# zxhuang1698/ShapeClipper

Hardware: AMD Instinct MI355X
Metric: train-step images/sec (Pix3D cfg, bs32/GPU) (higher is better)
Workload: dtype f32 (bf16x3-split MFMA, fp32 accumulate)

## Files before the change

shapeclipper_amd/csrc/conv3x3.hip:

```cpp
#include <hip/hip_runtime.h>

#include <map>
#include <mutex>
#include <tuple>
#include <vector>

#include "grid_cus.hpp"
#include "shapeclipper_hip.h"

#ifndef SC_CONV_SPANS
#define SC_CONV_SPANS 1
#endif
#ifndef SC_CONV_ABLATE
#define SC_CONV_ABLATE 0
#endif

namespace sc {

#ifdef SC_CONV_PROFILE
__device__ unsigned long long* conv_prof_buf = nullptr;
#define CV_STAMP(ID) { const unsigned long long t_ = __builtin_amdgcn_s_memrealtime(); if (conv_prof_buf && tid == 0) conv_prof_buf[(size_t)g * 32 + (ID)] = t_; }
#else
#define CV_STAMP(ID)
#endif

typedef float f32x16 __attribute__((ext_vector_type(16)));
typedef __bf16 cv_bf16x8 __attribute__((ext_vector_type(8)));
typedef __bf16 cv_bf16x2 __attribute__((ext_vector_type(2)));
typedef __attribute__((address_space(3))) void* lptr_cv_t;

__device__ __forceinline__ void conv_glds16(const void* gsrc, unsigned lds_dst) {
    unsigned keep;
    asm volatile("s_mov_b32 %0, m0\n\ts_mov_b32 m0, %2\n\ts_nop 0\n\tglobal_load_lds_dwordx4 %1, off\n\ts_mov_b32 m0, %0"
                 : "=&s"(keep) : "v"(gsrc), "s"(lds_dst) : "memory");
}

template <int W_, int CT_, int PT_, int WGM_, int WGN_, bool SPLIT_ = false, int S_ = 1, bool BD2_ = false>
struct ConvCfg {
    static constexpr int W = W_, CT = CT_, PT = PT_, WGM = WGM_, WGN = WGN_, CB = 8;
    static constexpr bool SPLIT = SPLIT_;
    static constexpr bool BD2 = BD2_;
    static constexpr int PSZ = 3 * 2 * CT * 4;
    static constexpr bool PAIRED = SPLIT && !BD2_;
    static_assert(!BD2 || (SPLIT && S_ == 1), "the stride-2 backward-data instance exists in the split arithmetic only");
    static constexpr int Wp = W + 2, HW = W * W, Sp = Wp * Wp;
    static constexpr int S = S_, WO = W / S, HWO = WO * WO;
    static constexpr int NT = 64 * WGM * WGN;
    static constexpr int WM = CT / (32 * WGM), WN = PT / (32 * WGN);
    static constexpr int WIMG = BD2 ? 2 * PSZ : (SPLIT ? 5 * PSZ : 9 * CB * CT);
    static constexpr int LMAX = S == 1 ? PT + 2 * (PT / W + 2) + 2 * Wp * (PT / HW + 1) + 2 * (Wp + 1)
                                       : S * PT + (PT / WO + 2) * S * (Wp - WO) + (PT / HWO + 1) * (Sp - S * (WO - 1) * (Wp + 1)) + 2 * (Wp + 1);
    static constexpr int LX = LMAX;
    static constexpr int NXE = (LMAX + NT - 1) / NT;
    static constexpr int STAGE = WIMG + (SPLIT ? 3 : 2) * LX * 4;
    static constexpr int LDS_BYTES = 2 * STAGE * 4;
    static constexpr int TILE = CT * PT;
    static constexpr int WGS_PER_CU = NT == 512 ? 1 : 2;
    static_assert(WM >= 1 && WN >= 1 && (NT == 512 || NT == 256) && LDS_BYTES * WGS_PER_CU <= 160 * 1024, "tile shape");
};

template <class C>
__device__ __forceinline__ int padded_q(int p) {
    const int b = p / C::HWO, r = p - b * C::HWO, y = r / C::WO, x = r - y * C::WO;
    return b * C::Sp + (C::S * y + 1) * C::Wp + (C::S * x + 1);
}

__host__ __device__ constexpr int bd2_pairs(int phase) { return phase == 3 ? 2 : 1; }
__host__ __device__ constexpr int bd2_pair_base(int phase) { return phase; }
__host__ __device__ constexpr int bd2_filter_tap(int phase, int pair, int h) {
    return phase == 0 ? (h == 0 ? 4 : -1)
         : phase == 1 ? (h == 0 ? 3 : 5)
         : phase == 2 ? (h == 0 ? 1 : 7)
         : pair == 0 ? (h == 0 ? 0 : 2) : (h == 0 ? 6 : 8);
}
__host__ __device__ constexpr int bd2_patch_tap(int phase, int pair, int h) {
    return phase == 0 ? 4
         : phase == 1 ? (h == 0 ? 5 : 4)
         : phase == 2 ? (h == 0 ? 7 : 4)
         : pair == 0 ? (h == 0 ? 8 : 7) : (h == 0 ? 5 : 4);
}

template <class C>
__host__ __device__ constexpr int conv_nk(int cin) { return C::PAIRED ? ((cin / C::CB + 1) & ~1) : cin / C::CB; }

struct ConvSplit {
    int rounds;
    int tail_tiles;
    int per_wg;
};
__host__ __device__ inline ConvSplit conv_split(int tiles, int nk, int G) {
    ConvSplit s;
    s.rounds = tiles / G;
    s.tail_tiles = tiles - s.rounds * G;
    s.per_wg = (int)(((long long)s.tail_tiles * nk + G - 1) / G);
    return s;
}

__device__ __forceinline__ long long conv_span_at(const int* __restrict__ spans, const ConvSplit& sp, int g, int nk) {
    return spans ? (long long)spans[g] : min((long long)g * sp.per_wg, (long long)sp.tail_tiles * nk);
}
__device__ __forceinline__ int conv_span_owner(const int* __restrict__ spans, const ConvSplit& sp, long long u, int G) {
    if (!spans) return (int)(u / sp.per_wg);
    int lo = 0, hi = G - 1;
    while (lo < hi) {
        const int mid = (lo + hi + 1) >> 1;
        if (spans[mid] <= u) lo = mid; else hi = mid - 1;
    }
    return lo;
}

template <class C>
__device__ __forceinline__ void conv_tile_decode(int tile, int nct, int& phase, int& pt, int& ct) {
    phase = C::BD2 ? tile & 3 : 0;
    const int t = C::BD2 ? tile >> 2 : tile;
    pt = t / nct, ct = t - pt * nct;
}
template <class C>
__device__ __forceinline__ float* conv_out_pixel(float* __restrict__ out, int p, int phase, int cout, int& cstride) {
    const int b = p / C::HWO, rem = p - b * C::HWO;
    if constexpr (C::BD2) {
        const int y = rem / C::W, x = rem - y * C::W;
        cstride = 4 * C::HW;
        return out + (size_t)b * cout * cstride + (2 * y + (phase >> 1)) * (2 * C::W) + 2 * x + (phase & 1);
    } else {
        cstride = C::HWO;
        return out + (size_t)b * cout * C::HWO + rem;
    }
}

template <class C>
__device__ __forceinline__ void conv_store_tile(float* __restrict__ out, const f32x16 (&acc)[C::WM][C::WN], int tile, int nct, int npix,
                                                int cout, int wm, int wn, int lane, const float* __restrict__ addend) {
    int phase, pt, ct;
    conv_tile_decode<C>(tile, nct, phase, pt, ct);
#pragma unroll
    for (int j = 0; j < C::WN; ++j) {
        const int p = pt * C::PT + (wn * C::WN + j) * 32 + (lane & 31);
        if (p >= npix) continue;
        int cs;
        float* ob = conv_out_pixel<C>(out, p, phase, cout, cs);
#pragma unroll
        for (int i = 0; i < C::WM; ++i)
#pragma unroll
            for (int r = 0; r < 16; ++r) {
                const int co = ct * C::CT + (wm * C::WM + i) * 32 + (r & 3) + 8 * (r >> 2) + 4 * (lane >> 5);
                if (co < cout) ob[(size_t)co * cs] = addend ? acc[i][j][r] + addend[(ob - out) + (size_t)co * cs] : acc[i][j][r];
            }
    }
}

template <class C>
__device__ __forceinline__ void conv_split_terms(const float4 (&a)[C::WM][3], const float4 (&b)[C::WN][3], f32x16 (&acc)[C::WM][C::WN]) {
#pragma unroll
    for (int term = 0; term < 6; ++term) {
        constexpr int PA[6] = {0, 2, 1, 0, 1, 0}, PB[6] = {2, 0, 1, 1, 0, 0};
#pragma unroll
        for (int i = 0; i < C::WM; ++i)
#pragma unroll
            for (int j = 0; j < C::WN; ++j)
#if SC_CONV_ABLATE & 1
                acc[i][j][term] += a[i][PA[term]].x * b[j][PB[term]].x;
#else
                acc[i][j] = __builtin_amdgcn_mfma_f32_32x32x16_bf16(__builtin_bit_cast(cv_bf16x8, a[i][PA[term]]),
                                                                    __builtin_bit_cast(cv_bf16x8, b[j][PB[term]]), acc[i][j], 0, 0, 0);
#endif
    }
}
template <class C, int PHASE>
__device__ __forceinline__ void conv_bd2_step(const float* Ws, const float* Xs, const int (&aoff)[C::WM], const int (&boff)[C::WN], int half,
                                              f32x16 (&acc)[C::WM][C::WN]) {
    constexpr int Wp = C::Wp, LX = C::LX, CT = C::CT;
#pragma unroll
    for (int tp = 0; tp < bd2_pairs(PHASE); ++tp) {
        constexpr int dummy = 0;
        (void)dummy;
        const int t0 = bd2_patch_tap(PHASE, tp, 0), t1 = bd2_patch_tap(PHASE, tp, 1);
        const int o0 = (t0 / 3) * Wp + t0 % 3, o1 = (t1 / 3) * Wp + t1 % 3;
        float4 a[C::WM][3], b[C::WN][3];
#pragma unroll
        for (int i = 0; i < C::WM; ++i)
#pragma unroll
            for (int pc = 0; pc < 3; ++pc) a[i][pc] = *reinterpret_cast<const float4*>(Ws + aoff[i] + (tp * 3 + pc) * 2 * CT * 4);
#pragma unroll
        for (int j = 0; j < C::WN; ++j)
#pragma unroll
            for (int pc = 0; pc < 3; ++pc)
                b[j][pc] = *reinterpret_cast<const float4*>(Xs + boff[j] + (pc * LX + o0) * 4 + half * (o1 - o0) * 4);
        conv_split_terms<C>(a, b, acc);
    }
}

template <class C>
__global__ __launch_bounds__(C::NT, C::WGS_PER_CU) void conv3x3_kernel(const float* __restrict__ x, const float* __restrict__ wpack,
                                                             float* __restrict__ out, float* __restrict__ partial, int batch, int cin,
                                                             int cout, const int* __restrict__ spans, const float* __restrict__ addend) {
    constexpr int W = C::W, Wp = C::Wp, HW = C::HW, Sp = C::Sp, CT = C::CT, PT = C::PT, CB = C::CB, NT = C::NT;
    constexpr int WM = C::WM, WN = C::WN, LX = C::LX, NXE = C::NXE;
    extern __shared__ float4 conv_smem[];
    float* S = reinterpret_cast<float*>(conv_smem);
    const int tid = threadIdx.x, lane = tid & 63, wave = tid >> 6, half = lane >> 5;
    const int wm = wave / C::WGN, wn = wave % C::WGN;
    const int npix = batch * C::HWO, nct = (cout + CT - 1) / CT, tiles = ((npix + PT - 1) / PT) * nct * (C::BD2 ? 4 : 1);
    const int nk = conv_nk<C>(cin), nk_real = cin / CB, G = gridDim.x, g = blockIdx.x;
    const ConvSplit sp = conv_split(tiles, nk, G);
    const int xq = G >> 3, xr = G & 7, xcd = g & 7;
    const int gperm = (xcd < xr ? xcd * (xq + 1) : xr * (xq + 1) + (xcd - xr) * xq) + (g >> 3);
    const long long unit_lo = conv_span_at(spans, sp, g, nk), unit_hi = conv_span_at(spans, sp, g + 1, nk);
    const unsigned lds0 = (unsigned)__builtin_amdgcn_readfirstlane((int)(unsigned)(size_t)(lptr_cv_t)S);
    const int wave_u = __builtin_amdgcn_readfirstlane(wave);

    CV_STAMP(0)
    for (int it = 0; it < sp.rounds + 2; ++it) {
        const int item = (C::WGS_PER_CU == 2 && g >= (G >> 1)) ? (it + sp.rounds) % (sp.rounds + 2) : it;
        int tile, kb0, kb1;
        if (item < sp.rounds) {
            tile = item * G + gperm, kb0 = 0, kb1 = nk;
        } else if (item == sp.rounds) {
            if (unit_lo >= unit_hi) continue;
            const int t = (int)(unit_lo / nk);
            tile = sp.rounds * G + t, kb0 = (int)(unit_lo - (long long)t * nk), kb1 = (int)min((long long)nk, unit_hi - (long long)t * nk);
        } else {
            const int t = (int)(unit_lo / nk) + 1;
            if (unit_lo >= unit_hi || (long long)t * nk >= unit_hi) continue;
            tile = sp.rounds * G + t, kb0 = 0, kb1 = (int)(unit_hi - (long long)t * nk);
        }
        int phase, pt, ct;
        conv_tile_decode<C>(tile, nct, phase, pt, ct);
        const int p0 = pt * PT;
        const int q0 = padded_q<C>(p0), q_lo = q0 - Wp - 1;

        int xoff[NXE];
#pragma unroll
        for (int i = 0; i < NXE; ++i) {
            const int e = tid + i * NT, q = q_lo + e;
            const int b = q / Sp, r = q - b * Sp, yp = r / Wp, xp = r - yp * Wp;
            const bool valid = e < C::LMAX && b < batch && yp >= 1 && yp <= W && xp >= 1 && xp <= W;
            xoff[i] = valid ? (b * cin * HW + (yp - 1) * W + (xp - 1)) : -1;
        }
        int boff[WN], aoff[WM];
#pragma unroll
        for (int j = 0; j < WN; ++j) {
            const int p = min(p0 + (wn * WN + j) * 32 + (lane & 31), npix - 1);
            boff[j] = (half * LX + padded_q<C>(p) - q0) * 4;
        }
#pragma unroll
        for (int i = 0; i < WM; ++i) aoff[i] = (half * CT + (wm * WM + i) * 32 + (lane & 31)) * 4;
        if constexpr (C::SPLIT) {
#pragma unroll
            for (int j = 0; j < WN; ++j) boff[j] -= half * LX * 4;
        }

        const int wimg = C::BD2 ? bd2_pairs(phase) * C::PSZ : C::WIMG;
        const float* wsrc = wpack + (C::BD2 ? (size_t)bd2_pair_base(phase) * nct * nk * C::PSZ : 0) +
                            (C::PAIRED ? (size_t)ct * (nk >> 1) * 9 * C::PSZ : (size_t)ct * nk * wimg);
        auto issue_w = [&](int kb, int stage) {
            const int CHUNKS = C::PAIRED ? ((kb & 1) ? 5 : 4) * C::PSZ / 4 : wimg / 4;
            const char* src = reinterpret_cast<const char*>(wsrc + (C::PAIRED ? ((size_t)(kb >> 1) * 9 + (kb & 1) * 4) * C::PSZ : (size_t)kb * wimg));
            const unsigned dst = lds0 + (unsigned)stage * (C::STAGE * 4);
#pragma unroll
            for (int c = 0; c < (C::WIMG / 4 + NT - 1) / NT; ++c) {
                const int chunk0 = c * NT + wave_u * 64;
                if (chunk0 + lane < CHUNKS) conv_glds16(src + (size_t)(chunk0 + lane) * 16, (unsigned)__builtin_amdgcn_readfirstlane((int)(dst + chunk0 * 16)));
            }
        };
        float xv[NXE][CB];
        unsigned xkeep = 0xffffffffu;
        const __amdgpu_buffer_rsrc_t xrs = __builtin_amdgcn_make_buffer_rsrc(
            const_cast<float*>(x), 0, (int)min((long long)batch * cin * HW * 4, 0x7fffffffLL), 0x00020000);
        int xoffb[NXE];
#pragma unroll
        for (int i = 0; i < NXE; ++i) xoffb[i] = xoff[i] >= 0 ? xoff[i] * 4 : (int)0x80000000;
        auto load_x = [&](int kb) {
            if constexpr (C::SPLIT) {
                xkeep = kb < nk_real ? 0xffffffffu : 0u;
#pragma unroll
                for (int i = 0; i < NXE; ++i)
#pragma unroll
                    for (int c = 0; c < CB; ++c)
                        xv[i][c] = __builtin_bit_cast(float, __builtin_amdgcn_raw_buffer_load_b32(xrs, xoffb[i], (kb * CB + c) * HW * 4, 0));
            } else {
                const float* xb = x + (size_t)kb * CB * HW;
#pragma unroll
                for (int i = 0; i < NXE; ++i)
#pragma unroll
                    for (int c = 0; c < CB; ++c) xv[i][c] = xoff[i] >= 0 ? xb[xoff[i] + c * HW] : 0.f;
            }
        };
        auto store_x = [&](int stage) {
            float4* Xs = reinterpret_cast<float4*>(S + stage * C::STAGE + C::WIMG);
#pragma unroll
            for (int i = 0; i < NXE; ++i) {
                const int e = tid + i * NT;
                if (e < C::LMAX) {
                    if constexpr (C::SPLIT) {
                        cv_bf16x8 p0, p1, p2;
#pragma unroll
                        for (int c = 0; c < CB; ++c) {
                            const float v = C::PAIRED ? __uint_as_float(__float_as_uint(xv[i][c]) & xkeep) : xv[i][c];
                            const __bf16 h0 = (__bf16)v;
                            const float r1 = v - (float)h0;
                            const __bf16 h1 = (__bf16)r1;
                            const float r2 = r1 - (float)h1;
                            p0[c] = h0, p1[c] = h1, p2[c] = (__bf16)r2;
                        }
                        Xs[e] = __builtin_bit_cast(float4, p0);
                        Xs[LX + e] = __builtin_bit_cast(float4, p1);
                        Xs[2 * LX + e] = __builtin_bit_cast(float4, p2);
                    } else {
                        Xs[e] = make_float4(xv[i][0], xv[i][1], xv[i][2], xv[i][3]);
                        Xs[LX + e] = make_float4(xv[i][4], xv[i][5], xv[i][6], xv[i][7]);
                    }
                }
            }
        };

        f32x16 acc[WM][WN];
#pragma unroll
        for (int i = 0; i < WM; ++i)
#pragma unroll
            for (int j = 0; j < WN; ++j)
#pragma unroll
                for (int r = 0; r < 16; ++r) acc[i][j][r] = 0.f;

        [[maybe_unused]] const int sid = 1 + 8 * (item < sp.rounds ? 0 : item - sp.rounds + 1);
        CV_STAMP(sid)
        asm volatile("s_waitcnt lgkmcnt(0)\n\ts_barrier" ::: "memory");
        if constexpr (C::PAIRED) {
            load_x(kb0 - (kb0 & 1));
            store_x(1);
        }
        issue_w(kb0, 0);
        load_x(kb0);
        store_x(0);
        CV_STAMP(sid + 1)
        for (int kb = kb0; kb < kb1; ++kb) {
            __builtin_amdgcn_s_waitcnt(0x0070);
            __builtin_amdgcn_s_barrier();
            const int st = (kb - kb0) & 1;
#ifdef SC_CONV_PROFILE
            if (kb == kb0 + 1) CV_STAMP(sid + 5)
#endif
#if SC_CONV_ABLATE & 12
            if (kb + 1 < kb1) {
                if (!(SC_CONV_ABLATE & 8)) issue_w(kb + 1, st ^ 1);
                if (!(SC_CONV_ABLATE & 4)) load_x(kb + 1);
            }
#else
            if (kb + 1 < kb1) { issue_w(kb + 1, st ^ 1); load_x(kb + 1); }
#endif
            const float* Ws = S + st * C::STAGE;
            const float* Xs = Ws + C::WIMG;
            if constexpr (C::BD2) {
                switch (phase) {
                    case 0: conv_bd2_step<C, 0>(Ws, Xs, aoff, boff, half, acc); break;
                    case 1: conv_bd2_step<C, 1>(Ws, Xs, aoff, boff, half, acc); break;
                    case 2: conv_bd2_step<C, 2>(Ws, Xs, aoff, boff, half, acc); break;
                    default: conv_bd2_step<C, 3>(Ws, Xs, aoff, boff, half, acc); break;
                }
            } else if constexpr (C::SPLIT) {
                float4 a[WM][3], b[WN][3];
                if (kb & 1) {
                    constexpr int o8 = 2 * Wp + 2;
                    const int xother = half ? 0 : (st ? -C::STAGE : C::STAGE);
#pragma unroll
                    for (int i = 0; i < WM; ++i)
#pragma unroll
                        for (int pc = 0; pc < 3; ++pc) a[i][pc] = *reinterpret_cast<const float4*>(Ws + aoff[i] + (4 * 3 + pc) * 2 * CT * 4);
#pragma unroll
                    for (int j = 0; j < WN; ++j)
#pragma unroll
                        for (int pc = 0; pc < 3; ++pc)
                            b[j][pc] = *reinterpret_cast<const float4*>(Xs + xother + boff[j] + (pc * LX + o8) * 4);
                    __builtin_amdgcn_s_waitcnt(0xc07f);
                    __builtin_amdgcn_s_barrier();
                    conv_split_terms<C>(a, b, acc);
                }
#pragma unroll
                for (int tp = 0; tp < 4; ++tp) {
                    const int t0 = 2 * tp, t1 = 2 * tp + 1;
                    const int o0 = (t0 / 3) * Wp + t0 % 3, o1 = (t1 / 3) * Wp + t1 % 3;
#if SC_CONV_ABLATE & 2
                    if (tp == 0 && kb == kb0)
#endif
                    {
#pragma unroll
                    for (int i = 0; i < WM; ++i)
#pragma unroll
                        for (int pc = 0; pc < 3; ++pc) a[i][pc] = *reinterpret_cast<const float4*>(Ws + aoff[i] + (tp * 3 + pc) * 2 * CT * 4);
#pragma unroll
                    for (int j = 0; j < WN; ++j)
#pragma unroll
                        for (int pc = 0; pc < 3; ++pc)
                            b[j][pc] = *reinterpret_cast<const float4*>(Xs + boff[j] + (pc * LX + o0) * 4 + half * (o1 - o0) * 4);
                    }
                    conv_split_terms<C>(a, b, acc);
                }
            } else {
            float4 a[2][WM], b[2][WN];
            auto frags = [&](int tap, float4 (&a2)[WM], float4 (&b2)[WN]) {
#pragma unroll
                for (int i = 0; i < WM; ++i) a2[i] = *reinterpret_cast<const float4*>(Ws + aoff[i] + tap * 2 * CT * 4);
#pragma unroll
                for (int j = 0; j < WN; ++j) b2[j] = *reinterpret_cast<const float4*>(Xs + boff[j] + ((tap / 3) * Wp + (tap % 3)) * 4);
            };
            frags(0, a[0], b[0]);
#pragma unroll
            for (int tap = 0; tap < 9; ++tap) {
                if (tap + 1 < 9) frags(tap + 1, a[(tap + 1) & 1], b[(tap + 1) & 1]);
#pragma unroll
                for (int s = 0; s < 4; ++s)
#pragma unroll
                    for (int i = 0; i < WM; ++i)
#pragma unroll
                        for (int j = 0; j < WN; ++j) {
                            const float av = s == 0 ? a[tap & 1][i].x : s == 1 ? a[tap & 1][i].y : s == 2 ? a[tap & 1][i].z : a[tap & 1][i].w;
                            const float bv = s == 0 ? b[tap & 1][j].x : s == 1 ? b[tap & 1][j].y : s == 2 ? b[tap & 1][j].z : b[tap & 1][j].w;
                            acc[i][j] = __builtin_amdgcn_mfma_f32_32x32x2f32(av, bv, acc[i][j], 0, 0, 0);
                        }
            }
            }
            if (kb + 1 < kb1 && !(SC_CONV_ABLATE & 4)) store_x(st ^ 1);
        }

        CV_STAMP(sid + 2)
        if (kb0 == 0 && kb1 == nk) {
            conv_store_tile<C>(out, acc, tile, nct, npix, cout, wm, wn, lane, addend);
        } else {
            float4* dst = reinterpret_cast<float4*>(partial + ((size_t)g * 2 + (item - sp.rounds)) * C::TILE);
#pragma unroll
            for (int i = 0; i < WM; ++i)
#pragma unroll
                for (int j = 0; j < WN; ++j)
#pragma unroll
                    for (int q = 0; q < 4; ++q) {
                        const float4 v = make_float4(acc[i][j][4 * q], acc[i][j][4 * q + 1], acc[i][j][4 * q + 2], acc[i][j][4 * q + 3]);
                        float4* d = dst + (((wave * WM + i) * WN + j) * 4 + q) * 64 + lane;
                        *d = v;
                    }
        }
#ifdef SC_CONV_PROFILE
        asm volatile("s_waitcnt vmcnt(0)" ::: "memory");
        CV_STAMP(sid + 3)
        if (conv_prof_buf && tid == 0) conv_prof_buf[(size_t)g * 32 + sid + 4] = (unsigned long long)(kb1 - kb0);
#endif
    }
    CV_STAMP(25)
}

template <class C>
__global__ __launch_bounds__(C::NT) void conv3x3_fixup_kernel(const float* __restrict__ partial, float* __restrict__ out, int batch,
                                                              int cin, int cout, int G, const int* __restrict__ spans,
                                                              const float* __restrict__ addend) {
    const int tid = threadIdx.x, lane = tid & 63, wave = tid >> 6;
    const int wm = wave / C::WGN, wn = wave % C::WGN;
    const int npix = batch * C::HWO, nct = (cout + C::CT - 1) / C::CT, tiles = ((npix + C::PT - 1) / C::PT) * nct * (C::BD2 ? 4 : 1);
    const int nk = conv_nk<C>(cin);
    const ConvSplit sp = conv_split(tiles, nk, G);
#ifdef SC_CONV_PROFILE
    if (conv_prof_buf && tid == 0) conv_prof_buf[(size_t)(8192 + blockIdx.x * 4 + blockIdx.y) * 2] = __builtin_amdgcn_s_memrealtime();
#endif
    const int t = blockIdx.x, r0 = 4 * blockIdx.y;
    const long long u0 = (long long)t * nk, u1 = u0 + nk;
    const int g_first = conv_span_owner(spans, sp, u0, G), g_last = conv_span_owner(spans, sp, u1 - 1, G);
    if (g_first == g_last && conv_span_at(spans, sp, g_first, nk) == u0 && conv_span_at(spans, sp, g_first + 1, nk) == u1) return;
    float acc[C::WM][C::WN][4];
#pragma unroll
    for (int i = 0; i < C::WM; ++i)
#pragma unroll
        for (int j = 0; j < C::WN; ++j)
#pragma unroll
            for (int r = 0; r < 4; ++r) acc[i][j][r] = 0.f;
    for (int g = g_first; g <= g_last; ++g) {
        const int which = (int)(conv_span_at(spans, sp, g, nk) / nk) == t ? 0 : 1;
        const float4* src = reinterpret_cast<const float4*>(partial + ((size_t)g * 2 + which) * C::TILE);
#pragma unroll
        for (int i = 0; i < C::WM; ++i)
#pragma unroll
            for (int j = 0; j < C::WN; ++j) {
                const float4 v = src[(((wave * C::WM + i) * C::WN + j) * 4 + (r0 >> 2)) * 64 + lane];
                acc[i][j][0] += v.x; acc[i][j][1] += v.y; acc[i][j][2] += v.z; acc[i][j][3] += v.w;
            }
    }
    const int tile = sp.rounds * G + t;
    int phase, pt, ct;
    conv_tile_decode<C>(tile, nct, phase, pt, ct);
#pragma unroll
    for (int j = 0; j < C::WN; ++j) {
        const int p = pt * C::PT + (wn * C::WN + j) * 32 + (lane & 31);
        if (p >= npix) continue;
        int cs;
        float* ob = conv_out_pixel<C>(out, p, phase, cout, cs);
#pragma unroll
        for (int i = 0; i < C::WM; ++i)
#pragma unroll
            for (int r = 0; r < 4; ++r) {
                const int co = ct * C::CT + (wm * C::WM + i) * 32 + r + 2 * r0 + 4 * (lane >> 5);
                if (co < cout) ob[(size_t)co * cs] = addend ? acc[i][j][r] + addend[(ob - out) + (size_t)co * cs] : acc[i][j][r];
            }
    }
#ifdef SC_CONV_PROFILE
    asm volatile("s_waitcnt vmcnt(0)" ::: "memory");
    if (conv_prof_buf && tid == 0) conv_prof_buf[(size_t)(8192 + blockIdx.x * 4 + blockIdx.y) * 2 + 1] = __builtin_amdgcn_s_memrealtime();
#endif
}

__device__ __forceinline__ float conv_w_at(const float* __restrict__ w, int cin, int cout, int co, int ci, int tap, int transpose_flip) {
    return transpose_flip ? w[((size_t)ci * cout + co) * 9 + (8 - tap)] : w[((size_t)co * cin + ci) * 9 + tap];
}
__device__ __forceinline__ unsigned conv_bf16_piece(float v, int pc) {
    const __bf16 h0 = (__bf16)v;
    const float r1 = v - (float)h0;
    const __bf16 h1 = (__bf16)r1;
    const __bf16 h2 = (__bf16)(r1 - (float)h1);
    const __bf16 h = pc == 0 ? h0 : pc == 1 ? h1 : h2;
    return (unsigned)__builtin_bit_cast(unsigned short, h);
}
__device__ __forceinline__ float conv_pack_word(const float* __restrict__ w, unsigned t, int CT, int nk, int cin, int cout, int flip,
                                                bool split) {
    if (!split) {
        const int s4 = (int)(t & 3);
        t >>= 2;
        const int cl = (int)(t % CT);
        t /= CT;
        const int h = (int)(t & 1);
        t >>= 1;
        const int tap = (int)(t % 9);
        t /= 9;
        const int kb = (int)(t % nk), ct = (int)(t / nk);
        const int ci = kb * 8 + 4 * h + s4, co = ct * CT + cl;
        return co < cout ? conv_w_at(w, cin, cout, co, ci, tap, flip) : 0.f;
    }
    const int wi = (int)(t & 3);
    t >>= 2;
    const int cl = (int)(t % CT);
    t /= CT;
    const int h = (int)(t & 1);
    t >>= 1;
    const int pc = (int)(t % 3);
    t /= 3;
    const int slot = (int)(t % 9);
    t /= 9;
    const int nkp = (nk + 1) >> 1, kp = (int)(t % nkp), ct = (int)(t / nkp);
    const int kb = 2 * kp + (slot < 4 ? 0 : (slot < 8 ? 1 : h)), tap = slot < 8 ? 2 * (slot & 3) + h : 8;
    const int co = ct * CT + cl, ci = kb * 8 + 2 * wi;
    unsigned lo = 0, hi = 0;
    if (kb < nk && co < cout) {
        lo = conv_bf16_piece(conv_w_at(w, cin, cout, co, ci, tap, flip), pc);
        hi = conv_bf16_piece(conv_w_at(w, cin, cout, co, ci + 1, tap, flip), pc);
    }
    return __uint_as_float(lo | (hi << 16));
}

template <class C>
__global__ void conv3x3_pack_bd2_kernel(const float* __restrict__ w, float* __restrict__ wpack, int cfwd_in, int cfwd_out) {
    const int nk = cfwd_out / C::CB, nct = (cfwd_in + C::CT - 1) / C::CT;
    const long long region = (long long)nct * nk * C::PSZ, total = 5 * region;
    for (long long i = (long long)blockIdx.x * blockDim.x + threadIdx.x; i < total; i += (long long)gridDim.x * blockDim.x) {
        const int r = (int)(i / region), phase = r < 3 ? r : 3;
        long long u = i - (long long)bd2_pair_base(phase) * region;
        const int blk = bd2_pairs(phase) * C::PSZ;
        const int ctkb = (int)(u / blk);
        u -= (long long)ctkb * blk;
        const int ct = ctkb / nk, kb = ctkb - ct * nk;
        const int pair = (int)(u / C::PSZ);
        int v = (int)(u - (long long)pair * C::PSZ);
        const int wi = v & 3;
        v >>= 2;
        const int cl = v % C::CT;
        v /= C::CT;
        const int h = v & 1, pc = v >> 1;
        const int tap = bd2_filter_tap(phase, pair, h), co_o = ct * C::CT + cl, ck = kb * 8 + 2 * wi;
        unsigned lo = 0, hi = 0;
        if (tap >= 0 && co_o < cfwd_in) {
            lo = conv_bf16_piece(w[((size_t)ck * cfwd_in + co_o) * 9 + tap], pc);
            hi = conv_bf16_piece(w[((size_t)(ck + 1) * cfwd_in + co_o) * 9 + tap], pc);
        }
        wpack[i] = __uint_as_float(lo | (hi << 16));
    }
}

template <class C>
__global__ void conv3x3_pack_kernel(const float* __restrict__ w, float* __restrict__ wpack, int cin, int cout, int transpose_flip) {
    const int nk = cin / C::CB, nct = (cout + C::CT - 1) / C::CT;
    const long long total = C::PAIRED ? (long long)nct * ((nk + 1) / 2) * 9 * C::PSZ : (long long)nct * nk * C::WIMG;
    for (long long i = (long long)blockIdx.x * blockDim.x + threadIdx.x; i < total; i += (long long)gridDim.x * blockDim.x)
        wpack[i] = conv_pack_word(w, (unsigned)i, C::CT, nk, cin, cout, transpose_flip, C::SPLIT);
}

using Conv56 = ConvCfg<56, 64, 512, 1, 8>;
using Conv28 = ConvCfg<28, 128, 256, 2, 4>;
using Conv14 = ConvCfg<14, 128, 256, 2, 4>;
using Conv7 = ConvCfg<7, 128, 128, 2, 4>;
using Conv56S2 = ConvCfg<56, 64, 256, 1, 8, false, 2>;
using Conv28S2 = ConvCfg<28, 64, 256, 1, 8, false, 2>;
using Conv14S2 = ConvCfg<14, 64, 256, 1, 8, false, 2>;
using Conv56S = ConvCfg<56, 64, 512, 1, 8, true>;
using Conv28S = ConvCfg<28, 64, 512, 1, 8, true>;
using Conv14S = ConvCfg<14, 64, 512, 1, 8, true>;
using Conv7S = ConvCfg<7, 64, 256, 1, 8, true>;
using Conv28BD = ConvCfg<28, 64, 512, 1, 8, true, 1, true>;
using Conv14BD = ConvCfg<14, 64, 512, 1, 8, true, 1, true>;
using Conv7BD = ConvCfg<7, 64, 256, 1, 8, true, 1, true>;

template <class C>
static long long pack_floats(int cin, int cout) {
    if (cin % C::CB) return -1;
    const long long nct = (cout + C::CT - 1) / C::CT, nk = cin / C::CB;
    return C::PAIRED ? nct * ((nk + 1) / 2) * 9 * C::PSZ : nct * nk * C::WIMG;
}

__global__ void conv3x3_pack_multi_kernel(const long long* __restrict__ table_g, int n, float* __restrict__ dst, long long total) {
    __shared__ long long table[128 * 6];
    for (int i = threadIdx.x; i < n * 6; i += blockDim.x) table[i] = table_g[i];
    __syncthreads();
    for (long long i = (long long)blockIdx.x * blockDim.x + threadIdx.x; i < total; i += (long long)gridDim.x * blockDim.x) {
        int lo = 0, hi = n - 1;
        while (lo < hi) {
            const int mid = (lo + hi + 1) >> 1;
            if (table[mid * 6 + 1] <= i) lo = mid; else hi = mid - 1;
        }
        const long long* row = table + lo * 6;
        const float* w = reinterpret_cast<const float*>(row[0]);
        const int cin = (int)row[2], cout = (int)row[3], CT = (int)row[4], flags = (int)row[5];
        dst[i] = conv_pack_word(w, (unsigned)(i - row[1]), CT, cin / 8, cin, cout, flags & 1, (flags & 2) != 0);
    }
}

__global__ __launch_bounds__(256) void conv3x3_pack_multi_split_kernel(const long long* __restrict__ table_g, int n, float* __restrict__ dst) {
    constexpr int CT = 64, UNIT = 9 * 3 * 2 * CT * 4, LST = 145;
    __shared__ float wl[CT * LST];
    __shared__ long long row_s[6];
    const int tid = threadIdx.x;
    const long long i0 = (long long)blockIdx.x * UNIT;
    if (tid == 0) {
        int lo = 0, hi = n - 1;
        while (lo < hi) {
            const int mid = (lo + hi + 1) >> 1;
            if (table_g[mid * 6 + 1] <= i0) lo = mid; else hi = mid - 1;
        }
        for (int k = 0; k < 6; ++k) row_s[k] = table_g[lo * 6 + k];
    }
    __syncthreads();
    const float* w = reinterpret_cast<const float*>(row_s[0]);
    const int cin = (int)row_s[2], cout = (int)row_s[3], flip = (int)row_s[5] & 1, nkp = (cin / 8 + 1) / 2;
    const int unit = (int)((i0 - row_s[1]) / UNIT), ct = unit / nkp, kp = unit - ct * nkp;
    for (int e = tid; e < 16 * CT * 9; e += 256) {
        int cl, sc, tap;
        float v = 0.f;
        if (flip) {
            sc = e / (CT * 9);
            const int r = e - sc * (CT * 9);
            cl = r / 9; tap = 8 - (r - cl * 9);
            if (ct * CT + cl < cout && kp * 16 + sc < cin) v = w[((size_t)(kp * 16 + sc) * cout + ct * CT) * 9 + r];
        } else {
            cl = e / 144;
            const int r = e - cl * 144;
            sc = r / 9; tap = r - sc * 9;
            if (ct * CT + cl < cout && kp * 16 + sc < cin) v = w[((size_t)(ct * CT + cl) * cin + kp * 16) * 9 + r];
        }
        wl[cl * LST + sc * 9 + tap] = v;
    }
    __syncthreads();
    for (int v = tid; v < UNIT; v += 256) {
        const int wi = v & 3, cl = (v >> 2) & 63, h = (v >> 8) & 1, q = v >> 9, pc = q % 3, slot = q / 3;
        const int kl = slot < 4 ? 0 : (slot < 8 ? 1 : h), tap = slot < 8 ? 2 * (slot & 3) + h : 8;
        const unsigned lo = conv_bf16_piece(wl[cl * LST + (8 * kl + 2 * wi) * 9 + tap], pc);
        const unsigned hi = conv_bf16_piece(wl[cl * LST + (8 * kl + 2 * wi + 1) * 9 + tap], pc);
        dst[i0 + v] = __uint_as_float(lo | (hi << 16));
    }
}

static int conv_grid() { return grid_cus(); }

template <class C>
static long long workspace_floats() { return (long long)conv_grid() * C::WGS_PER_CU * 2 * C::TILE; }

template <class C>
static int launch_pack(const float* w, float* wpack, int cin, int cout, int tf, hipStream_t st) {
    if (cin % C::CB) return (int)hipErrorInvalidValue;
    const long long total = pack_floats<C>(cin, cout);
    hipLaunchKernelGGL((conv3x3_pack_kernel<C>), dim3((unsigned)((total + 255) / 256 < 2048 ? (total + 255) / 256 : 2048)), dim3(256), 0, st,
                       w, wpack, cin, cout, tf);
    return (int)hipGetLastError();
}

struct SpanTable {
    int* dev = nullptr;
    std::vector<int> host;
};
static std::mutex span_mu;
static std::map<std::tuple<int, int, int, int, int>, SpanTable> span_cache;

static const int* conv_spans(int tail_tiles, int nk, int G, int ov2, hipStream_t st) {
    std::map<std::tuple<int, int, int, int, int>, SpanTable>& cache = span_cache;
    int dev = 0;
    (void)hipGetDevice(&dev);
    std::lock_guard<std::mutex> lock(span_mu);
    const auto key = std::make_tuple(dev, tail_tiles, nk, G, ov2);
    auto it = cache.find(key);
    if (it != cache.end()) return it->second.dev;
    hipStreamCaptureStatus cap = hipStreamCaptureStatusNone;
    if (hipStreamIsCapturing(st, &cap) != hipSuccess || cap != hipStreamCaptureStatusNone) {
        (void)hipGetLastError();
        return nullptr;
    }
    const int total = tail_tiles * nk;
    std::vector<int> U(G + 1), best;
    auto build = [&](int bound) {
        int pos = 0;
        for (int g = 0; g < G; ++g) {
            U[g] = pos;
            int end = pos;
            while (end < total && end - pos < nk) {
                const int e1 = end + 1, items = (e1 - 1) / nk - pos / nk + 1;
                if (end > pos && 2 * (e1 - pos) + ov2 * items > bound) break;
                end = e1;
            }
            pos = end;
        }
        U[G] = total;
        return pos >= total;
    };
    int lo = 2 * ((total + G - 1) / G), hi = lo + 4 * ov2 + 4;
    while (!build(hi)) hi += 2 * nk;
    while (lo < hi) {
        const int mid = (lo + hi) / 2;
        if (build(mid)) hi = mid; else lo = mid + 1;
    }
    (void)build(hi);
    SpanTable& t = cache[key];
    t.host = U;
    if (hipMalloc(&t.dev, (size_t)(G + 1) * sizeof(int)) != hipSuccess ||
        hipMemcpyAsync(t.dev, t.host.data(), (size_t)(G + 1) * sizeof(int), hipMemcpyHostToDevice, st) != hipSuccess ||
        hipStreamSynchronize(st) != hipSuccess) {
        (void)hipGetLastError();
        if (t.dev) (void)hipFree(t.dev);
        t.dev = nullptr;
    }
    return t.dev;
}

template <class C>
static int launch_conv(const float* x, const float* wpack, float* out, float* workspace, int batch, int cin, int cout, hipStream_t st,
                       const float* addend = nullptr) {
    if (cin % C::CB || batch <= 0) return (int)hipErrorInvalidValue;
    const int tiles = ((batch * C::HWO + C::PT - 1) / C::PT) * ((cout + C::CT - 1) / C::CT) * (C::BD2 ? 4 : 1), nk = conv_nk<C>(cin);
    const int G = conv_grid() * C::WGS_PER_CU;
    if (C::SPLIT && (long long)batch * cin * C::HW * 4 > 0x7fffffffLL) return (int)hipErrorInvalidValue;
    (void)hipFuncSetAttribute((const void*)conv3x3_kernel<C>, hipFuncAttributeMaxDynamicSharedMemorySize, C::LDS_BYTES);
    const ConvSplit sp = conv_split(tiles, nk, G);
    const int* spans = (SC_CONV_SPANS && sp.tail_tiles > 0 && sp.per_wg <= nk) ? conv_spans(sp.tail_tiles, nk, G, C::PT >= 512 ? 2 : 3, st) : nullptr;
    hipLaunchKernelGGL((conv3x3_kernel<C>), dim3(G), dim3(C::NT), C::LDS_BYTES, st, x, wpack, out, workspace, batch, cin, cout, spans, addend);
    if (sp.tail_tiles > 0)
        hipLaunchKernelGGL((conv3x3_fixup_kernel<C>), dim3(sp.tail_tiles, 4), dim3(C::NT), 0, st, workspace, out, batch, cin, cout, G, spans, addend);
    return (int)hipGetLastError();
}

}

extern "C" int sc_conv3x3_release_tables(void) {
    std::lock_guard<std::mutex> lock(sc::span_mu);
    int dev0 = 0;
    (void)hipGetDevice(&dev0);
    for (auto& kv : sc::span_cache)
        if (kv.second.dev) {
            (void)hipSetDevice(std::get<0>(kv.first));
            (void)hipFree(kv.second.dev);
        }
    sc::span_cache.clear();
    (void)hipSetDevice(dev0);
    return 0;
}

#define SC_CONV_DISPATCH(hw, CALL)                   \
    switch (hw) {                                    \
        case 56: return CALL(sc::Conv56);            \
        case 28: return CALL(sc::Conv28);            \
        case 14: return CALL(sc::Conv14);            \
        case 7: return CALL(sc::Conv7);              \
        default: return -1;                          \
    }

#define SC_CONV_DISPATCH_SPLIT(hw, CALL)              \
    switch (hw) {                                    \
        case 56: return CALL(sc::Conv56S);           \
        case 28: return CALL(sc::Conv28S);           \
        case 14: return CALL(sc::Conv14S);           \
        case 7: return CALL(sc::Conv7S);             \
        default: return -1;                          \
    }

#define SC_CONV_DISPATCH_S2(hw, CALL)                 \
    switch (hw) {                                    \
        case 56: return CALL(sc::Conv56S2);          \
        case 28: return CALL(sc::Conv28S2);          \
        case 14: return CALL(sc::Conv14S2);          \
        default: return -1;                          \
    }

#define SC_CONV_DISPATCH_BD(hw, CALL)                 \
    switch (hw) {                                    \
        case 56: return CALL(sc::Conv28BD);          \
        case 28: return CALL(sc::Conv14BD);          \
        case 14: return CALL(sc::Conv7BD);           \
        default: return -1;                          \
    }
#ifdef SC_CONV_PROFILE
extern "C" int sc_conv_debug_set_prof(unsigned long long* buf) {
    return (int)hipMemcpyToSymbol(HIP_SYMBOL(sc::conv_prof_buf), &buf, sizeof(buf));
}
#endif
extern "C" long long sc_conv3x3s2_bd_pack_floats(int cin, int cout, int hw) {
#define CALL(C) (cout % C::CB ? -1 : 5LL * ((cin + C::CT - 1) / C::CT) * (cout / C::CB) * C::PSZ)
    SC_CONV_DISPATCH_BD(hw, CALL)
#undef CALL
}
extern "C" long long sc_conv3x3s2_bd_workspace_floats(int hw) {
#define CALL(C) sc::workspace_floats<C>()
    SC_CONV_DISPATCH_BD(hw, CALL)
#undef CALL
}
namespace sc {
template <class C>
static int launch_pack_bd2(const float* w, float* wpack, int cin, int cout, hipStream_t st) {
    if (cout % C::CB) return (int)hipErrorInvalidValue;
    const long long total = 5LL * ((cin + C::CT - 1) / C::CT) * (cout / C::CB) * C::PSZ;
    hipLaunchKernelGGL((conv3x3_pack_bd2_kernel<C>), dim3((unsigned)((total + 255) / 256 < 2048 ? (total + 255) / 256 : 2048)), dim3(256), 0, st,
                       w, wpack, cin, cout);
    return (int)hipGetLastError();
}
}
extern "C" int sc_conv3x3s2_bd_pack(const float* w, float* w_pack, int cin, int cout, int hw, void* stream) {
#define CALL(C) sc::launch_pack_bd2<C>(w, w_pack, cin, cout, (hipStream_t)stream)
    SC_CONV_DISPATCH_BD(hw, CALL)
#undef CALL
}
extern "C" int sc_conv3x3s2_backward_data(const float* gy, const float* w_pack, float* gx, float* workspace, int batch, int cin, int cout,
                                          int hw, void* stream) {
#define CALL(C) sc::launch_conv<C>(gy, w_pack, gx, workspace, batch, cout, cin, (hipStream_t)stream)
    SC_CONV_DISPATCH_BD(hw, CALL)
#undef CALL
}

extern "C" long long sc_conv3x3s2_pack_floats(int cin, int cout, int hw) {
#define CALL(C) sc::pack_floats<C>(cin, cout)
    SC_CONV_DISPATCH_S2(hw, CALL)
#undef CALL
}
extern "C" long long sc_conv3x3s2_workspace_floats(int hw) {
#define CALL(C) sc::workspace_floats<C>()
    SC_CONV_DISPATCH_S2(hw, CALL)
#undef CALL
}
extern "C" int sc_conv3x3s2_forward(const float* x, const float* w_pack, float* out, float* workspace, int batch, int cin, int cout, int hw,
                                    void* stream) {
#define CALL(C) sc::launch_conv<C>(x, w_pack, out, workspace, batch, cin, cout, (hipStream_t)stream)
    SC_CONV_DISPATCH_S2(hw, CALL)
#undef CALL
}

extern "C" long long sc_conv3x3_pack_floats_split(int cin, int cout, int hw) {
#define CALL(C) sc::pack_floats<C>(cin, cout)
    SC_CONV_DISPATCH_SPLIT(hw, CALL)
#undef CALL
}
extern "C" long long sc_conv3x3_workspace_floats_split(int hw) {
#define CALL(C) sc::workspace_floats<C>()
    SC_CONV_DISPATCH_SPLIT(hw, CALL)
#undef CALL
}
extern "C" int sc_conv3x3_tile_channels_split(int hw) {
#define CALL(C) C::CT
    SC_CONV_DISPATCH_SPLIT(hw, CALL)
#undef CALL
}
extern "C" int sc_conv3x3_forward_split(const float* x, const float* w_pack, float* out, float* workspace, int batch, int cin, int cout,
                                        int hw, void* stream) {
#define CALL(C) sc::launch_conv<C>(x, w_pack, out, workspace, batch, cin, cout, (hipStream_t)stream)
    SC_CONV_DISPATCH_SPLIT(hw, CALL)
#undef CALL
}

extern "C" long long sc_conv3x3_pack_floats(int cin, int cout, int hw) {
#define CALL(C) sc::pack_floats<C>(cin, cout)
    SC_CONV_DISPATCH(hw, CALL)
#undef CALL
}

extern "C" long long sc_conv3x3_workspace_floats(int hw) {
#define CALL(C) sc::workspace_floats<C>()
    SC_CONV_DISPATCH(hw, CALL)
#undef CALL
}

extern "C" int sc_conv3x3_tile_channels(int hw) {
#define CALL(C) C::CT
    SC_CONV_DISPATCH(hw, CALL)
#undef CALL
}

extern "C" int sc_conv3x3_pack_multi_units(const long long* table, int n, float* dst, long long total, void* stream) {
    if (n <= 0 || total <= 0) return 0;
    if (n > 128 || total % 13824) return (int)hipErrorInvalidValue;
    hipLaunchKernelGGL(sc::conv3x3_pack_multi_split_kernel, dim3((unsigned)(total / 13824)), dim3(256), 0, (hipStream_t)stream, table, n, dst);
    return (int)hipGetLastError();
}

extern "C" int sc_conv3x3_pack_multi(const long long* table, int n, float* dst, long long total, void* stream) {
    if (n <= 0 || total <= 0) return 0;
    if (n > 128) return (int)hipErrorInvalidValue;
    const long long blocks = (total + 255) / 256;
    hipLaunchKernelGGL(sc::conv3x3_pack_multi_kernel, dim3((unsigned)(blocks < 8192 ? blocks : 8192)), dim3(256), 0, (hipStream_t)stream, table, n, dst,
                       total);
    return (int)hipGetLastError();
}

extern "C" int sc_conv3x3_pack(const float* w, float* w_pack, int cin, int cout, int hw, int transpose_flip, void* stream) {
    if (transpose_flip & 4) {
#define CALL(C) sc::launch_pack<C>(w, w_pack, cin, cout, transpose_flip & 1, (hipStream_t)stream)
        SC_CONV_DISPATCH_S2(hw, CALL)
#undef CALL
    }
    if (transpose_flip & 2) {
#define CALL(C) sc::launch_pack<C>(w, w_pack, cin, cout, transpose_flip & 1, (hipStream_t)stream)
        SC_CONV_DISPATCH_SPLIT(hw, CALL)
#undef CALL
    }
#define CALL(C) sc::launch_pack<C>(w, w_pack, cin, cout, transpose_flip & 1, (hipStream_t)stream)
    SC_CONV_DISPATCH(hw, CALL)
#undef CALL
}

extern "C" int sc_conv3x3_forward_add(const float* x, const float* w_pack, const float* addend, float* out, float* workspace, int batch, int cin,
                                      int cout, int hw, int split, void* stream) {
    if (split) {
#define CALL(C) sc::launch_conv<C>(x, w_pack, out, workspace, batch, cin, cout, (hipStream_t)stream, addend)
        SC_CONV_DISPATCH_SPLIT(hw, CALL)
#undef CALL
    }
#define CALL(C) sc::launch_conv<C>(x, w_pack, out, workspace, batch, cin, cout, (hipStream_t)stream, addend)
    SC_CONV_DISPATCH(hw, CALL)
#undef CALL
}

extern "C" int sc_conv3x3_forward(const float* x, const float* w_pack, float* out, float* workspace, int batch, int cin, int cout, int hw,
                                  void* stream) {
#define CALL(C) sc::launch_conv<C>(x, w_pack, out, workspace, batch, cin, cout, (hipStream_t)stream)
    SC_CONV_DISPATCH(hw, CALL)
#undef CALL
}
```

Baseline: 1015.

## Compute all four stride-2 backward-data phases per tile sharing one input stage

The stride-2 backward-data conv kernel now computes all four output phases in one work tile, with four accumulator sets fed from a single staged input window. The tile count drops by four and each input load is reused four times. The tile shape becomes 128 pixels with a 2x4 wave grid, stores go out as float2 pairs, and the weight loader pulls all tap-pair images per k-block. When tail tiles fit whole per workgroup, a trivial span table is used and the fixup kernel is skipped. This raises register pressure from four accumulator sets and changes the partial workspace layout.

Result: no change. 1005 (-1.0%).

```diff
diff --git a/shapeclipper_amd/csrc/conv3x3.hip b/shapeclipper_amd/csrc/conv3x3.hip
--- a/shapeclipper_amd/csrc/conv3x3.hip
+++ b/shapeclipper_amd/csrc/conv3x3.hip
@@ -47,14 +47,15 @@
     static constexpr int S = S_, WO = W / S, HWO = WO * WO;
     static constexpr int NT = 64 * WGM * WGN;
     static constexpr int WM = CT / (32 * WGM), WN = PT / (32 * WGN);
-    static constexpr int WIMG = BD2 ? 2 * PSZ : (SPLIT ? 5 * PSZ : 9 * CB * CT);
+    static constexpr int WIMG = SPLIT ? 5 * PSZ : 9 * CB * CT;
+    static constexpr int NPH = BD2 ? 4 : 1;
     static constexpr int LMAX = S == 1 ? PT + 2 * (PT / W + 2) + 2 * Wp * (PT / HW + 1) + 2 * (Wp + 1)
                                        : S * PT + (PT / WO + 2) * S * (Wp - WO) + (PT / HWO + 1) * (Sp - S * (WO - 1) * (Wp + 1)) + 2 * (Wp + 1);
     static constexpr int LX = LMAX;
     static constexpr int NXE = (LMAX + NT - 1) / NT;
     static constexpr int STAGE = WIMG + (SPLIT ? 3 : 2) * LX * 4;
     static constexpr int LDS_BYTES = 2 * STAGE * 4;
-    static constexpr int TILE = CT * PT;
+    static constexpr int TILE = NPH * CT * PT;
     static constexpr int WGS_PER_CU = NT == 512 ? 1 : 2;
     static_assert(WM >= 1 && WN >= 1 && (NT == 512 || NT == 256) && LDS_BYTES * WGS_PER_CU <= 160 * 1024, "tile shape");
 };
@@ -109,19 +110,16 @@
     return lo;
 }
 
-template <class C>
-__device__ __forceinline__ void conv_tile_decode(int tile, int nct, int& phase, int& pt, int& ct) {
-    phase = C::BD2 ? tile & 3 : 0;
-    const int t = C::BD2 ? tile >> 2 : tile;
-    pt = t / nct, ct = t - pt * nct;
-}
-template <class C>
-__device__ __forceinline__ float* conv_out_pixel(float* __restrict__ out, int p, int phase, int cout, int& cstride) {
+__device__ __forceinline__ void conv_tile_decode(int tile, int nct, int& pt, int& ct) {
+    pt = tile / nct, ct = tile - pt * nct;
+}
+template <class C>
+__device__ __forceinline__ float* conv_out_pixel(float* __restrict__ out, int p, int cout, int& cstride) {
     const int b = p / C::HWO, rem = p - b * C::HWO;
     if constexpr (C::BD2) {
         const int y = rem / C::W, x = rem - y * C::W;
         cstride = 4 * C::HW;
-        return out + (size_t)b * cout * cstride + (2 * y + (phase >> 1)) * (2 * C::W) + 2 * x + (phase & 1);
+        return out + (size_t)b * cout * cstride + (2 * y) * (2 * C::W) + 2 * x;
     } else {
         cstride = C::HWO;
         return out + (size_t)b * cout * C::HWO + rem;
@@ -129,22 +127,36 @@
 }
 
 template <class C>
-__device__ __forceinline__ void conv_store_tile(float* __restrict__ out, const f32x16 (&acc)[C::WM][C::WN], int tile, int nct, int npix,
+__device__ __forceinline__ void conv_store_tile(float* __restrict__ out, const f32x16 (&acc)[C::NPH][C::WM][C::WN], int tile, int nct, int npix,
                                                 int cout, int wm, int wn, int lane, const float* __restrict__ addend) {
-    int phase, pt, ct;
-    conv_tile_decode<C>(tile, nct, phase, pt, ct);
+    int pt, ct;
+    conv_tile_decode(tile, nct, pt, ct);
 #pragma unroll
     for (int j = 0; j < C::WN; ++j) {
         const int p = pt * C::PT + (wn * C::WN + j) * 32 + (lane & 31);
         if (p >= npix) continue;
         int cs;
-        float* ob = conv_out_pixel<C>(out, p, phase, cout, cs);
+        float* ob = conv_out_pixel<C>(out, p, cout, cs);
 #pragma unroll
         for (int i = 0; i < C::WM; ++i)
 #pragma unroll
             for (int r = 0; r < 16; ++r) {
                 const int co = ct * C::CT + (wm * C::WM + i) * 32 + (r & 3) + 8 * (r >> 2) + 4 * (lane >> 5);
-                if (co < cout) ob[(size_t)co * cs] = addend ? acc[i][j][r] + addend[(ob - out) + (size_t)co * cs] : acc[i][j][r];
+                if (co >= cout) continue;
+                if constexpr (C::BD2) {
+#pragma unroll
+                    for (int py = 0; py < 2; ++py) {
+                        float2* o2 = reinterpret_cast<float2*>(ob + (size_t)co * cs + py * 2 * C::W);
+                        float2 v = make_float2(acc[2 * py][i][j][r], acc[2 * py + 1][i][j][r]);
+                        if (addend) {
+                            const float2 ad = *reinterpret_cast<const float2*>(addend + (reinterpret_cast<float*>(o2) - out));
+                            v.x += ad.x, v.y += ad.y;
+                        }
+                        *o2 = v;
+                    }
+                } else {
+                    ob[(size_t)co * cs] = addend ? acc[0][i][j][r] + addend[(ob - out) + (size_t)co * cs] : acc[0][i][j][r];
+                }
             }
     }
 }
@@ -200,7 +212,7 @@
     float* S = reinterpret_cast<float*>(conv_smem);
     const int tid = threadIdx.x, lane = tid & 63, wave = tid >> 6, half = lane >> 5;
     const int wm = wave / C::WGN, wn = wave % C::WGN;
-    const int npix = batch * C::HWO, nct = (cout + CT - 1) / CT, tiles = ((npix + PT - 1) / PT) * nct * (C::BD2 ? 4 : 1);
+    const int npix = batch * C::HWO, nct = (cout + CT - 1) / CT, tiles = ((npix + PT - 1) / PT) * nct;
     const int nk = conv_nk<C>(cin), nk_real = cin / CB, G = gridDim.x, g = blockIdx.x;
     const ConvSplit sp = conv_split(tiles, nk, G);
     const int xq = G >> 3, xr = G & 7, xcd = g & 7;
@@ -224,8 +236,8 @@
             if (unit_lo >= unit_hi || (long long)t * nk >= unit_hi) continue;
             tile = sp.rounds * G + t, kb0 = 0, kb1 = (int)(unit_hi - (long long)t * nk);
         }
-        int phase, pt, ct;
-        conv_tile_decode<C>(tile, nct, phase, pt, ct);
+        int pt, ct;
+        conv_tile_decode(tile, nct, pt, ct);
         const int p0 = pt * PT;
         const int q0 = padded_q<C>(p0), q_lo = q0 - Wp - 1;
 
@@ -250,9 +262,9 @@
             for (int j = 0; j < WN; ++j) boff[j] -= half * LX * 4;
         }
 
-        const int wimg = C::BD2 ? bd2_pairs(phase) * C::PSZ : C::WIMG;
-        const float* wsrc = wpack + (C::BD2 ? (size_t)bd2_pair_base(phase) * nct * nk * C::PSZ : 0) +
-                            (C::PAIRED ? (size_t)ct * (nk >> 1) * 9 * C::PSZ : (size_t)ct * nk * wimg);
+        const int wimg = C::WIMG;
+        const float* wsrc = wpack + (C::PAIRED ? (size_t)ct * (nk >> 1) * 9 * C::PSZ : (C::BD2 ? (size_t)0 : (size_t)ct * nk * wimg));
+        [[maybe_unused]] const size_t bd2_region = (size_t)nct * nk * C::PSZ;
         auto issue_w = [&](int kb, int stage) {
             const int CHUNKS = C::PAIRED ? ((kb & 1) ? 5 : 4) * C::PSZ / 4 : wimg / 4;
             const char* src = reinterpret_cast<const char*>(wsrc + (C::PAIRED ? ((size_t)(kb >> 1) * 9 + (kb & 1) * 4) * C::PSZ : (size_t)kb * wimg));
@@ -260,7 +272,16 @@
 #pragma unroll
             for (int c = 0; c < (C::WIMG / 4 + NT - 1) / NT; ++c) {
                 const int chunk0 = c * NT + wave_u * 64;
-                if (chunk0 + lane < CHUNKS) conv_glds16(src + (size_t)(chunk0 + lane) * 16, (unsigned)__builtin_amdgcn_readfirstlane((int)(dst + chunk0 * 16)));
+                if constexpr (C::BD2) {
+                    static_assert((C::PSZ / 4) % 64 == 0, "a wave's 64 chunks must not straddle two tap-pair images");
+                    constexpr int IC = C::PSZ / 4;
+                    const int img = chunk0 / IC, ctkb = ct * nk + kb;
+                    const float* s = img < 3 ? wpack + (size_t)img * bd2_region + (size_t)ctkb * C::PSZ + (size_t)(chunk0 - img * IC) * 4
+                                             : wpack + 3 * bd2_region + (size_t)ctkb * 2 * C::PSZ + (size_t)(chunk0 - 3 * IC) * 4;
+                    if (chunk0 < CHUNKS) conv_glds16(reinterpret_cast<const char*>(s) + (size_t)lane * 16, (unsigned)__builtin_amdgcn_readfirstlane((int)(dst + chunk0 * 16)));
+                } else {
+                    if (chunk0 + lane < CHUNKS) conv_glds16(src + (size_t)(chunk0 + lane) * 16, (unsigned)__builtin_amdgcn_readfirstlane((int)(dst + chunk0 * 16)));
+                }
             }
         };
         float xv[NXE][CB];
@@ -314,13 +335,16 @@
             }
         };
 
-        f32x16 acc[WM][WN];
-#pragma unroll
-        for (int i = 0; i < WM; ++i)
-#pragma unroll
-            for (int j = 0; j < WN; ++j)
-#pragma unroll
-                for (int r = 0; r < 16; ++r) acc[i][j][r] = 0.f;
+        f32x16 accs[C::NPH][WM][WN];
+        f32x16 (&acc)[WM][WN] = accs[0];
+#pragma unroll
+        for (int ph = 0; ph < C::NPH; ++ph)
+#pragma unroll
+            for (int i = 0; i < WM; ++i)
+#pragma unroll
+                for (int j = 0; j < WN; ++j)
+#pragma unroll
+                    for (int r = 0; r < 16; ++r) accs[ph][i][j][r] = 0.f;
 
         [[maybe_unused]] const int sid = 1 + 8 * (item < sp.rounds ? 0 : item - sp.rounds + 1);
         CV_STAMP(sid)
@@ -351,12 +375,10 @@
             const float* Ws = S + st * C::STAGE;
             const float* Xs = Ws + C::WIMG;
             if constexpr (C::BD2) {
-                switch (phase) {
-                    case 0: conv_bd2_step<C, 0>(Ws, Xs, aoff, boff, half, acc); break;
-                    case 1: conv_bd2_step<C, 1>(Ws, Xs, aoff, boff, half, acc); break;
-                    case 2: conv_bd2_step<C, 2>(Ws, Xs, aoff, boff, half, acc); break;
-                    default: conv_bd2_step<C, 3>(Ws, Xs, aoff, boff, half, acc); break;
-                }
+                conv_bd2_step<C, 0>(Ws + bd2_pair_base(0) * C::PSZ, Xs, aoff, boff, half, accs[0]);
+                conv_bd2_step<C, 1>(Ws + bd2_pair_base(1) * C::PSZ, Xs, aoff, boff, half, accs[1]);
+                conv_bd2_step<C, 2>(Ws + bd2_pair_base(2) * C::PSZ, Xs, aoff, boff, half, accs[2]);
+                conv_bd2_step<C, 3>(Ws + bd2_pair_base(3) * C::PSZ, Xs, aoff, boff, half, accs[3]);
             } else if constexpr (C::SPLIT) {
                 float4 a[WM][3], b[WN][3];
                 if (kb & 1) {
@@ -424,17 +446,19 @@
 
         CV_STAMP(sid + 2)
         if (kb0 == 0 && kb1 == nk) {
-            conv_store_tile<C>(out, acc, tile, nct, npix, cout, wm, wn, lane, addend);
+            conv_store_tile<C>(out, accs, tile, nct, npix, cout, wm, wn, lane, addend);
         } else {
             float4* dst = reinterpret_cast<float4*>(partial + ((size_t)g * 2 + (item - sp.rounds)) * C::TILE);
 #pragma unroll
+            for (int ph = 0; ph < C::NPH; ++ph)
+#pragma unroll
             for (int i = 0; i < WM; ++i)
 #pragma unroll
                 for (int j = 0; j < WN; ++j)
 #pragma unroll
                     for (int q = 0; q < 4; ++q) {
-                        const float4 v = make_float4(acc[i][j][4 * q], acc[i][j][4 * q + 1], acc[i][j][4 * q + 2], acc[i][j][4 * q + 3]);
-                        float4* d = dst + (((wave * WM + i) * WN + j) * 4 + q) * 64 + lane;
+                        const float4 v = make_float4(accs[ph][i][j][4 * q], accs[ph][i][j][4 * q + 1], accs[ph][i][j][4 * q + 2], accs[ph][i][j][4 * q + 3]);
+                        float4* d = dst + ((((wave * C::NPH + ph) * WM + i) * WN + j) * 4 + q) * 64 + lane;
                         *d = v;
                     }
         }
@@ -453,7 +477,7 @@
                                                               const float* __restrict__ addend) {
     const int tid = threadIdx.x, lane = tid & 63, wave = tid >> 6;
     const int wm = wave / C::WGN, wn = wave % C::WGN;
-    const int npix = batch * C::HWO, nct = (cout + C::CT - 1) / C::CT, tiles = ((npix + C::PT - 1) / C::PT) * nct * (C::BD2 ? 4 : 1);
+    const int npix = batch * C::HWO, nct = (cout + C::CT - 1) / C::CT, tiles = ((npix + C::PT - 1) / C::PT) * nct;
     const int nk = conv_nk<C>(cin);
     const ConvSplit sp = conv_split(tiles, nk, G);
 #ifdef SC_CONV_PROFILE
@@ -463,39 +487,57 @@
     const long long u0 = (long long)t * nk, u1 = u0 + nk;
     const int g_first = conv_span_owner(spans, sp, u0, G), g_last = conv_span_owner(spans, sp, u1 - 1, G);
     if (g_first == g_last && conv_span_at(spans, sp, g_first, nk) == u0 && conv_span_at(spans, sp, g_first + 1, nk) == u1) return;
-    float acc[C::WM][C::WN][4];
+    float acc[C::NPH][C::WM][C::WN][4];
+#pragma unroll
+    for (int ph = 0; ph < C::NPH; ++ph)
 #pragma unroll
     for (int i = 0; i < C::WM; ++i)
 #pragma unroll
         for (int j = 0; j < C::WN; ++j)
 #pragma unroll
-            for (int r = 0; r < 4; ++r) acc[i][j][r] = 0.f;
+            for (int r = 0; r < 4; ++r) acc[ph][i][j][r] = 0.f;
     for (int g = g_first; g <= g_last; ++g) {
         const int which = (int)(conv_span_at(spans, sp, g, nk) / nk) == t ? 0 : 1;
         const float4* src = reinterpret_cast<const float4*>(partial + ((size_t)g * 2 + which) * C::TILE);
 #pragma unroll
+        for (int ph = 0; ph < C::NPH; ++ph)
+#pragma unroll
         for (int i = 0; i < C::WM; ++i)
 #pragma unroll
             for (int j = 0; j < C::WN; ++j) {
-                const float4 v = src[(((wave * C::WM + i) * C::WN + j) * 4 + (r0 >> 2)) * 64 + lane];
-                acc[i][j][0] += v.x; acc[i][j][1] += v.y; acc[i][j][2] += v.z; acc[i][j][3] += v.w;
+                const float4 v = src[((((wave * C::NPH + ph) * C::WM + i) * C::WN + j) * 4 + (r0 >> 2)) * 64 + lane];
+                acc[ph][i][j][0] += v.x; acc[ph][i][j][1] += v.y; acc[ph][i][j][2] += v.z; acc[ph][i][j][3] += v.w;
             }
     }
     const int tile = sp.rounds * G + t;
-    int phase, pt, ct;
-    conv_tile_decode<C>(tile, nct, phase, pt, ct);
+    int pt, ct;
+    conv_tile_decode(tile, nct, pt, ct);
 #pragma unroll
     for (int j = 0; j < C::WN; ++j) {
         const int p = pt * C::PT + (wn * C::WN + j) * 32 + (lane & 31);
         if (p >= npix) continue;
         int cs;
-        float* ob = conv_out_pixel<C>(out, p, phase, cout, cs);
+        float* ob = conv_out_pixel<C>(out, p, cout, cs);
 #pragma unroll
         for (int i = 0; i < C::WM; ++i)
 #pragma unroll
             for (int r = 0; r < 4; ++r) {
                 const int co = ct * C::CT + (wm * C::WM + i) * 32 + r + 2 * r0 + 4 * (lane >> 5);
-                if (co < cout) ob[(size_t)co * cs] = addend ? acc[i][j][r] + addend[(ob - out) + (size_t)co * cs] : acc[i][j][r];
+                if (co >= cout) continue;
+                if constexpr (C::BD2) {
+#pragma unroll
+                    for (int py = 0; py < 2; ++py) {
+                        float2* o2 = reinterpret_cast<float2*>(ob + (size_t)co * cs + py * 2 * C::W);
+                        float2 v = make_float2(acc[2 * py][i][j][r], acc[2 * py + 1][i][j][r]);
+                        if (addend) {
+                            const float2 ad = *reinterpret_cast<const float2*>(addend + (reinterpret_cast<float*>(o2) - out));
+                            v.x += ad.x, v.y += ad.y;
+                        }
+                        *o2 = v;
+                    }
+                } else {
+                    ob[(size_t)co * cs] = addend ? acc[0][i][j][r] + addend[(ob - out) + (size_t)co * cs] : acc[0][i][j][r];
+                }
             }
     }
 #ifdef SC_CONV_PROFILE
@@ -598,9 +640,9 @@
 using Conv28S = ConvCfg<28, 64, 512, 1, 8, true>;
 using Conv14S = ConvCfg<14, 64, 512, 1, 8, true>;
 using Conv7S = ConvCfg<7, 64, 256, 1, 8, true>;
-using Conv28BD = ConvCfg<28, 64, 512, 1, 8, true, 1, true>;
-using Conv14BD = ConvCfg<14, 64, 512, 1, 8, true, 1, true>;
-using Conv7BD = ConvCfg<7, 64, 256, 1, 8, true, 1, true>;
+using Conv28BD = ConvCfg<28, 64, 128, 2, 4, true, 1, true>;
+using Conv14BD = ConvCfg<14, 64, 128, 2, 4, true, 1, true>;
+using Conv7BD = ConvCfg<7, 64, 128, 2, 4, true, 1, true>;
 
 template <class C>
 static long long pack_floats(int cin, int cout) {
@@ -706,6 +748,9 @@
     }
     const int total = tail_tiles * nk;
     std::vector<int> U(G + 1), best;
+    if (ov2 < 0) {
+        for (int g = 0; g <= G; ++g) U[g] = g < tail_tiles ? g * nk : total;
+    } else {
     auto build = [&](int bound) {
         int pos = 0;
         for (int g = 0; g < G; ++g) {
@@ -728,6 +773,7 @@
         if (build(mid)) hi = mid; else lo = mid + 1;
     }
     (void)build(hi);
+    }
     SpanTable& t = cache[key];
     t.host = U;
     if (hipMalloc(&t.dev, (size_t)(G + 1) * sizeof(int)) != hipSuccess ||
@@ -744,14 +790,15 @@
 static int launch_conv(const float* x, const float* wpack, float* out, float* workspace, int batch, int cin, int cout, hipStream_t st,
                        const float* addend = nullptr) {
     if (cin % C::CB || batch <= 0) return (int)hipErrorInvalidValue;
-    const int tiles = ((batch * C::HWO + C::PT - 1) / C::PT) * ((cout + C::CT - 1) / C::CT) * (C::BD2 ? 4 : 1), nk = conv_nk<C>(cin);
+    const int tiles = ((batch * C::HWO + C::PT - 1) / C::PT) * ((cout + C::CT - 1) / C::CT), nk = conv_nk<C>(cin);
     const int G = conv_grid() * C::WGS_PER_CU;
     if (C::SPLIT && (long long)batch * cin * C::HW * 4 > 0x7fffffffLL) return (int)hipErrorInvalidValue;
     (void)hipFuncSetAttribute((const void*)conv3x3_kernel<C>, hipFuncAttributeMaxDynamicSharedMemorySize, C::LDS_BYTES);
     const ConvSplit sp = conv_split(tiles, nk, G);
-    const int* spans = (SC_CONV_SPANS && sp.tail_tiles > 0 && sp.per_wg <= nk) ? conv_spans(sp.tail_tiles, nk, G, C::PT >= 512 ? 2 : 3, st) : nullptr;
+    const bool whole = C::BD2 && SC_CONV_SPANS && sp.tail_tiles > 0 && nk <= sp.per_wg + 8;
+    const int* spans = (SC_CONV_SPANS && sp.tail_tiles > 0 && sp.per_wg <= nk) ? conv_spans(sp.tail_tiles, nk, G, whole ? -1 : (C::PT >= 512 ? 2 : 3), st) : nullptr;
     hipLaunchKernelGGL((conv3x3_kernel<C>), dim3(G), dim3(C::NT), C::LDS_BYTES, st, x, wpack, out, workspace, batch, cin, cout, spans, addend);
-    if (sp.tail_tiles > 0)
+    if (sp.tail_tiles > 0 && !(whole && spans))
         hipLaunchKernelGGL((conv3x3_fixup_kernel<C>), dim3(sp.tail_tiles, 4), dim3(C::NT), 0, st, workspace, out, batch, cin, cout, G, spans, addend);
     return (int)hipGetLastError();
 }
```
